# xbpeng/DeepMimic

Measured on NVIDIA H100. Metric: env-steps/sec (30 Hz policy steps; humanoid3d_spinkick, 4096 envs/GPU), higher is better.
Workload: dtype f32

## Files before the change

deepmimic_b200/capi.py:

```python
import ctypes as C
import os

import numpy as np

_REPO = os.path.dirname(os.path.dirname(os.path.abspath(__file__)))
_LIB_PATH = os.environ.get("DM_LIB", os.path.join(_REPO, "deepmimic_b200", "libdeepmimic_b200.so"))
_lib = None


class DmDims(C.Structure):
    _fields_ = [(n, C.c_int) for n in ("num_envs", "num_joints", "pose_dim", "num_dofs", "state_size", "goal_size", "action_size", "snapshot_size",
                                        "updates_per_action", "num_update_substeps")] + [("motion_duration", C.c_double), ("amp_obs_size", C.c_int)]


_fp = C.POINTER(C.c_float)


class DmMlpGatedWeights(C.Structure):
    _fields_ = ([(n, C.c_int) for n in ("in_dim", "goal_dim", "h0", "h1", "out_dim", "gate_common", "gate_hidden")]
                + [(n, _fp) for n in ("w0", "b0", "w1", "b1", "w2", "b2", "gc_w", "gc_b")]
                + [(n, _fp * 2) for n in ("gh_w", "gh_b", "gs_w", "gs_b", "gb_w", "gb_b")]
                + [(n, _fp) for n in ("s_mean", "s_std", "g_mean", "g_std", "a_mean", "a_std")] + [("s_clip", C.c_float), ("g_clip", C.c_float)])


# ... 14 lines not shown
                + [(n, C.c_float) for n in ("stepsize", "momentum", "weight_decay", "logit_reg_weight", "grad_penalty_weight")] + [("stats", C.c_void_p)])


class DmLearnGatedNet(C.Structure):
    _fields_ = [(n, C.c_void_p * 10) for n in ("w", "b", "acc_w", "acc_b")]


class DmLearnGatedBatch(C.Structure):
    _anonymous_ = ("batch",)
    _fields_ = [("batch", DmLearnBatch), ("goals", C.c_void_p), ("g_mean", C.c_void_p), ("g_istd", C.c_void_p), ("g_clip", C.c_float)]


DM_STATE_OFFSET, DM_STATE_SCALE, DM_ACTION_OFFSET, DM_ACTION_SCALE, DM_ACTION_BOUND_MIN, DM_ACTION_BOUND_MAX, DM_STATE_NORM_GROUPS = range(7)

EXPORTS = ["dm_create", "dm_load_host", "dm_plan_launch", "dm_get_model_info", "dm_get_link_table", "dm_destroy", "dm_last_error", "dm_get_dims", "dm_get_static", "dm_get_scene_name", "dm_stream", "dm_sync", "dm_set_mode", "dm_set_sample_count", "dm_get_time_limits", "dm_reset", "dm_set_action",
           "dm_update", "dm_set_env_order", "dm_plan_env_order", "dm_get_env_order", "dm_record_state", "dm_record_goal", "dm_goal_host", "dm_reset_clips", "dm_record_amp_obs_expert_clips", "dm_get_clip_table", "dm_get_task_state", "dm_set_task_state", "dm_get_task_params", "dm_calc_reward", "dm_calc_reward_imitate", "dm_record_amp_obs_agent", "dm_record_amp_obs_expert", "dm_amp_obs_host", "dm_sample_amp_obs_expert", "dm_expert_sample_count", "dm_observe", "dm_get_flags", "dm_step_host", "dm_step_host_reset", "dm_set_time_limits", "dm_exchange_create", "dm_exchange_connect", "dm_exchange_publish", "dm_exchange_acquire", "dm_exchange_release", "dm_exchange_status", "dm_exchange_destroy", "dm_set_timing", "dm_step_host_timing", "dm_get_snapshot",
           "dm_set_snapshot", "dm_state_size", "dm_save_state", "dm_load_state", "dm_get_counters", "dm_get_section_profile", "dm_mlp_create", "dm_mlp_forward", "dm_mlp_create_gated", "dm_mlp_forward_gated",
           "dm_mlp_forward_style_reward", "dm_mlp_launches", "dm_mlp_destroy", "dm_td_lambda_returns", "dm_mlp_set_weights_device", "dm_learn_create",
           "dm_mlp_set_normalizers_device", "dm_learn_set_weights", "dm_learn_step", "dm_learn_disc_step", "dm_learn_destroy",
           "dm_learn_create_gated", "dm_learn_set_gated_weights", "dm_learn_gated_step", "dm_mlp_set_gated_weights_device", "dm_mlp_set_gated_normalizers_device"]


def lib():
    global _lib
    if _lib is None:
        if not os.path.exists(_LIB_PATH):
            raise RuntimeError("deepmimic_b200: %s is missing -- run `python -c 'import __graft_entry__ as g; g.build()'`. "
                               "There is no CPU fallback." % _LIB_PATH)
        L = C.CDLL(_LIB_PATH)
        vp, dp, fp, ip = C.c_void_p, C.POINTER(C.c_double), C.c_void_p, C.c_void_p
        L.dm_create.restype = vp
# ... 8 lines not shown
        L.dm_get_dims.argtypes = [vp, C.POINTER(DmDims)]
        L.dm_get_static.argtypes = [vp, C.c_int, dp]
        L.dm_get_scene_name.argtypes = [vp, C.c_char_p, C.c_int]
        L.dm_stream.restype = vp
        L.dm_stream.argtypes = [vp]
        L.dm_sync.argtypes = [vp]
        L.dm_set_mode.argtypes = [vp, C.c_int]
        L.dm_set_sample_count.argtypes = [vp, C.c_longlong]
        L.dm_get_time_limits.argtypes = [vp, dp]
        L.dm_reset.argtypes = [vp, C.c_int, dp, dp, dp]
        L.dm_set_action.argtypes = [vp, fp]
        L.dm_update.argtypes = [vp, C.c_double, C.c_int]
        L.dm_set_env_order.argtypes = [vp, C.c_int]
        L.dm_plan_env_order.argtypes = [C.POINTER(C.c_int), C.c_int, C.c_int, C.c_int, C.POINTER(C.c_int)]
        L.dm_get_env_order.argtypes = [vp, C.POINTER(C.c_int), C.POINTER(C.c_int), C.POINTER(C.c_int)]
        L.dm_record_state.argtypes = [vp, fp]
        L.dm_record_goal.argtypes = [vp, fp]
        L.dm_calc_reward.argtypes = [vp, fp]
        L.dm_calc_reward_imitate.argtypes = [vp, fp]
        L.dm_goal_host.argtypes = [vp, fp]
        L.dm_reset_clips.argtypes = [vp, C.c_int, C.POINTER(C.c_int), dp, dp, dp]
        L.dm_record_amp_obs_expert_clips.argtypes = [vp, C.POINTER(C.c_int), dp, fp]
        L.dm_get_clip_table.argtypes = [vp, C.POINTER(C.c_int), dp, dp]
        L.dm_get_task_state.argtypes = [vp, C.c_int, dp]
        L.dm_set_task_state.argtypes = [vp, C.c_int, dp]
        L.dm_get_task_params.argtypes = [vp, dp, C.POINTER(C.c_uint64)]
        L.dm_record_amp_obs_agent.argtypes = [vp, fp]
        L.dm_record_amp_obs_expert.argtypes = [vp, dp, fp]
        L.dm_amp_obs_host.argtypes = [vp, C.c_int, dp, fp]
        L.dm_sample_amp_obs_expert.argtypes = [vp, C.c_int, vp, vp, vp]
# ... 150 lines not shown

    def update(self, dt, n_updates=1):
        self._chk(lib().dm_update(self.h, dt, n_updates))

    def set_env_order(self, on):
        self._chk(lib().dm_set_env_order(self.h, 1 if on else 0))

    def env_order(self):
        ip = C.POINTER(C.c_int)
        plan = np.zeros(3, dtype=np.int32)
        self._chk(lib().dm_get_env_order(self.h, plan.ctypes.data_as(ip), None, None))
        keys, order = np.zeros(plan[0], dtype=np.int32), np.zeros(plan[0], dtype=np.int32)
        self._chk(lib().dm_get_env_order(self.h, plan.ctypes.data_as(ip), keys.ctypes.data_as(ip), order.ctypes.data_as(ip)))
        return keys, order, int(plan[1]), int(plan[2])

    def observe(self, state=None, reward=None):
        self._chk(lib().dm_observe(self.h, C.c_void_p(state.data_ptr()) if state is not None else None,
                                   C.c_void_p(reward.data_ptr()) if reward is not None else None))

    def reward_imitate(self, out):
        self._chk(lib().dm_calc_reward_imitate(self.h, C.c_void_p(out.data_ptr())))

    def record_goal(self, out):
        self._chk(lib().dm_record_goal(self.h, C.c_void_p(out.data_ptr())))

    def goal_host(self):
        out = np.zeros((self.num_envs, self.dims.goal_size), dtype=np.float32)
        self._chk(lib().dm_goal_host(self.h, C.c_void_p(out.ctypes.data)))
        return out

# ... 121 lines not shown

    def load_state(self, buf):
        b = np.ascontiguousarray(buf, dtype=np.uint8)
        if b.ndim != 1 or b.size < 24 or int(b[16:24].view(np.uint64)[0]) != b.size:
            raise ValueError("load_state: not a complete save_state() blob (%s bytes)" % (b.shape,))
        self._chk(lib().dm_load_state(self.h, C.c_void_p(b.ctypes.data)))

    def counters(self):
        out = (C.c_int64 * 2)()
        self._chk(lib().dm_get_counters(self.h, out))
        return int(out[0]), int(out[1])

    def section_profile(self):
        nb, nw = C.c_int(0), C.c_int(0)
        self._chk(lib().dm_get_section_profile(self.h, None, C.byref(nb), C.byref(nw)))
        out = np.zeros((nb.value, nw.value, 18), dtype=np.uint32)
        self._chk(lib().dm_get_section_profile(self.h, C.c_void_p(out.ctypes.data), None, None))
        return out

    def stream(self):
        return lib().dm_stream(self.h)


class HostModel:
    INFO = dict(parents=0, joint_types=1, dof_offsets=2, pose_offsets=3, fall_bodies=4, end_effectors=5)

    def __init__(self, args, asset_root):
        L = lib()
        enc = [a.encode() for a in args]
        arr = (C.c_char_p * len(enc))(*enc)
        h = L.dm_load_host(asset_root.encode(), len(enc), arr)
# ... 282 lines not shown
```

deepmimic_b200/csrc/capi.cu:

```cuda
#include <cuda_runtime.h>

#include <algorithm>
#include <map>
#include <mutex>
#include <cmath>
#include <cstddef>
#include <cstdio>
#include <cstdlib>
#include <numeric>
#include <cstring>
#include <ctime>
#include <utility>
#include <memory>
#include <string>
#include <vector>

#include "../../include/deepmimic_b200.h"
#include "host/assets.hpp"
#include "kernels/dm_model.cuh"

namespace dmk {
__global__ void dm_flags_kernel(DevState st, int32_t* out, int num_real_envs) {
    int e = blockIdx.x * blockDim.x + threadIdx.x;
    if (e >= num_real_envs) return;
// ... 52 lines not shown
    double* d_frame_times = nullptr;
    float* d_frames = nullptr;
    float* d_frame_vel = nullptr;
    double* d_inj[3] = {nullptr, nullptr, nullptr};
    int32_t* d_flags4 = nullptr;
    float *d_amp = nullptr, *p_amp = nullptr;
    float *d_goal = nullptr, *p_goal = nullptr;
    dmk::ClipTable ctab{};
    dmk::ClipTable* d_ctab = nullptr; int* d_clip_inj = nullptr;
    int total_frames = 0;
    float *d_act = nullptr, *d_obs = nullptr, *d_rew = nullptr;
    float *p_act = nullptr, *p_obs = nullptr, *p_rew = nullptr; int32_t* p_flags = nullptr;
    cudaStream_t stream = nullptr;
    int device = 0, num_envs = 0, padded_envs = 0, W = 32, tiles = 2, maxrows = 36, smem_bytes = 0, mode = 0;
    int* d_order = nullptr;
    dmk::StepLayout lay{};
    uint64_t seed = 0, env_offset = 0;
    int64_t launches = 0;
    uint64_t amp_calls = 0;
    uint64_t expert_samples = 0;
    std::vector<double> st_off, st_scale, act_off, act_scale, act_min, act_max, st_groups;
    std::vector<std::pair<const void*, bool>> pin_cache;
    int x_rank = 0, x_world = 0;
    char* x_base = nullptr;
    char* x_peer[8] = {nullptr, nullptr, nullptr, nullptr, nullptr, nullptr, nullptr, nullptr};
    size_t x_data_off = 0, x_parity_bytes = 0;
    bool timing = false;
    cudaEvent_t tev[5] = {nullptr, nullptr, nullptr, nullptr, nullptr};
    double host_ms[3] = {0, 0, 0};
    std::vector<void*> dev_bufs, pinned_bufs;
// ... 222 lines not shown

int launch_step(dm_handle* h, double dt, int n_updates) {
    const dmk::StepKernel kern = dmk::kStepKernels[tile_index(h)][task_scene(h)];
    static std::mutex mu;
    static std::map<std::pair<int, const void*>, int> configured;
    {
        std::lock_guard<std::mutex> lock(mu);
        int& have = configured[{h->device, reinterpret_cast<const void*>(kern)}];
        if (h->smem_bytes > have) {
            DM_CUDA(cudaFuncSetAttribute(kern, cudaFuncAttributeMaxDynamicSharedMemorySize, h->smem_bytes));
            DM_CUDA(cudaFuncSetAttribute(kern, cudaFuncAttributePreferredSharedMemoryCarveout, 100));
            DM_CUDA(cudaFuncSetAttribute(dmk::dm_env_order_kernel, cudaFuncAttributePreferredSharedMemoryCarveout, 100));
            have = h->smem_bytes;
        }
    }
    if (h->st.order) {
        dmk::dm_env_order_kernel<<<1, dmk::kEnvOrderThreads, 0, h->stream>>>(h->st.load, h->padded_envs, h->tiles, h->W, h->d_order);
        if (launched(h)) return 1;
    }
    kern<<<h->padded_envs / h->tiles, h->tiles * h->W, h->smem_bytes, h->stream>>>(h->d_model, h->st, h->d_frame_times, h->d_frames, dt, n_updates,
                                                                                   h->sa.cfg.num_sim_substeps, h->lay);
    return launched(h);
}
int launch_observe_fan(dm_handle* h, const dmk::ObsFan& fan) {
    const dmk::ObserveKernel kern = dmk::kObserveKernels[tile_index(h)][task_scene(h)];
    const size_t smem = static_cast<size_t>(dmk::kPolicyBlock / h->W) * h->hm.state_size * sizeof(float);
    kern<<<policy_grid(h), dmk::kPolicyBlock, smem, h->stream>>>(h->d_model, h->st, h->d_frame_times, h->d_frames, h->d_frame_vel, fan, h->num_envs);
    return launched(h);
}
int launch_observe(dm_handle* h, float* d_state, float* d_reward) {
    dmk::ObsFan fan{};
    fan.n = 1; fan.obs[0] = d_state; fan.rew[0] = d_reward; fan.done[0] = nullptr;
    return launch_observe_fan(h, fan);
}
int launch_reset(dm_handle* h, int force, const double* kt, const double* mt, const double* th, const int* clip) {
    const dmk::ResetKernel kern = dmk::kResetKernels[tile_index(h)][task_scene(h)];
// ... 71 lines not shown
    auto even_split = [&](int slots, int cap) {
        const int waves = ((num_envs + cap - 1) / cap + slots - 1) / slots;
        int t = std::min(cap, std::max(min_tiles, (num_envs + waves * slots - 1) / (waves * slots)));
        if (H.W == 16 && (t & 1)) t = (t + 1 <= cap) ? t + 1 : t - 1;
        return std::make_pair(waves, t);
    };
    auto [waves, tiles] = even_split(sms, max_tiles);
    {
        const int cap2 = std::min({max_tiles, (smem_sm / 2 - smem_reserved - hot) / per_env, 65536 / (2 * regs * H.W)});
        if (cap2 >= min_tiles) {
            const auto [waves2, tiles2] = even_split(2 * sms, cap2);
            if (waves2 < waves) { waves = waves2; tiles = tiles2; }
        }
    }
    H.tiles = tiles;
    const int quantum = (tiles * (64 / H.W)) / std::__gcd(tiles, 64 / H.W);
    H.padded_envs = ((num_envs + quantum - 1) / quantum) * quantum;
    H.smem_bytes = dmk::dm_step_smem_bytes(H.lay, H.tiles) + 1024;
    return true;
}

extern "C" {

const char* dm_last_error(void) { return g_err.c_str(); }
void dm_set_last_error(const char* msg) { g_err = msg ? msg : ""; }

static bool load_host_model(dm_handle& H, const char* asset_root, int argc, const char** argv) {
    try {
        std::vector<std::string> args(argv, argv + argc);
        dmh::ArgParser ap;
// ... 109 lines not shown
        h->ctab.cdf[c] = h->sa.clip_cdf[c];
        ci.is_getup = std::find(h->sa.cfg.getup_motion_ids.begin(), h->sa.cfg.getup_motion_ids.end(), static_cast<int>(c)) != h->sa.cfg.getup_motion_ids.end() ? 1 : 0;
        h->total_frames += mc.num_frames;
    }
    const size_t TF = static_cast<size_t>(h->total_frames);
    DM_CUDA(cudaStreamCreateWithFlags(&h->stream, cudaStreamNonBlocking));
    if (alloc_buffer(h, &h->d_model, 1) || alloc_buffer(h, &h->st.sim, N * ss) || alloc_buffer(h, &h->st.time, N * dmk::kTimeDoubles, kZeroed) ||
        alloc_buffer(h, &h->st.flags, N * dmk::kFlagInts, kZeroed) || alloc_buffer(h, &h->st.manifold, N * M.nl * dmk::kManifoldFloats, kZeroed) ||
        alloc_buffer(h, &h->d_frame_times, TF) || alloc_buffer(h, &h->d_frames, TF * M.pose_dim) || alloc_buffer(h, &h->d_frame_vel, TF * M.pose_dim) ||
        alloc_buffer(h, &h->d_flags4, N * 4) || alloc_buffer(h, &h->d_amp, N * M.amp_obs_size) || alloc_buffer(h, &h->p_amp, N * M.amp_obs_size, kPinned) ||
        alloc_buffer(h, &h->st.hist, N * 2 * M.pose_dim, kZeroed) || alloc_buffer(h, &h->d_act, N * std::max(1, M.action_size)) ||
        alloc_buffer(h, &h->d_obs, N * M.state_size) || alloc_buffer(h, &h->d_rew, N) || alloc_buffer(h, &h->p_act, N * std::max(1, M.action_size), kPinned) ||
        alloc_buffer(h, &h->p_obs, N * M.state_size, kPinned) || alloc_buffer(h, &h->p_rew, N, kPinned) || alloc_buffer(h, &h->p_flags, N * 4, kPinned))
        return 1;
    for (auto& p : h->d_inj) if (alloc_buffer(h, &p, N)) return 1;
    if (alloc_buffer(h, &h->st.load, N) || alloc_buffer(h, &h->d_order, N)) return 1;
    {
        std::vector<int> load(N, 0), ident(N);
        std::fill(load.begin() + h->num_envs, load.end(), dmk::kLoadPadding);
        std::iota(ident.begin(), ident.end(), 0);
        DM_CUDA(cudaMemcpy(h->st.load, load.data(), N * sizeof(int), cudaMemcpyHostToDevice));
        DM_CUDA(cudaMemcpy(h->d_order, ident.data(), N * sizeof(int), cudaMemcpyHostToDevice));
    }
    h->st.order = (h->W == 16) ? h->d_order : nullptr;
#ifdef DM_PROFILE
    if (alloc_buffer(h, &h->st.prof, static_cast<size_t>(h->padded_envs / h->tiles) * (h->tiles * h->W / 32) * dmk::kProfCounters, kZeroed)) return 1;
#endif
    h->st.num_envs = h->padded_envs; h->st.num_real = h->num_envs;
    if (task_scene(h)) {
        if (alloc_buffer(h, &h->st.task, N * dmk::kTaskDoubles, kZeroed) || alloc_buffer(h, &h->st.taskx, N * dmk::kTaskExtDoubles, kZeroed) ||
            alloc_buffer(h, &h->d_goal, N * 4) || alloc_buffer(h, &h->p_goal, N * 4, kPinned) || alloc_buffer(h, &h->st.clip, N, kZeroed) ||
            alloc_buffer(h, &h->d_clip_inj, N) || alloc_buffer(h, &h->d_ctab, 1))
            return 1;
        DM_CUDA(cudaMemcpy(h->d_ctab, &h->ctab, sizeof(dmk::ClipTable), cudaMemcpyHostToDevice));
    }
    h->st.ctab = h->d_ctab;
    std::vector<float> frames(TF * M.pose_dim), fvel(frames.size());
    std::vector<double> ftimes(TF);
    for (size_t c = 0; c < h->sa.clips.size(); ++c) {
        const dmh::MotionClip& mc = h->sa.clips[c];
        const std::vector<double> fv = build_frame_vel(h->sa.character, mc);
// ... 147 lines not shown
        return fail();
    }
    std::vector<int> sorted(n_padded);
    std::iota(sorted.begin(), sorted.end(), 0);
    std::stable_sort(sorted.begin(), sorted.end(), [&](int a, int b) { return dmk::env_load_bucket(keys[a]) < dmk::env_load_bucket(keys[b]); });
    for (int r = 0; r < n_padded; ++r) order[dmk::env_order_slot(r, n_padded, tiles, W)] = sorted[r];
    return 0;
}
int dm_get_env_order(dm_handle* h, int* h_plan3, int* h_keys, int* h_order) {
    DM_DEVICE(h);
    if (h_plan3) { h_plan3[0] = h->padded_envs; h_plan3[1] = h->tiles; h_plan3[2] = h->W; }
    DM_CUDA(cudaStreamSynchronize(h->stream));
    if (h_keys) DM_CUDA(cudaMemcpy(h_keys, h->st.load, sizeof(int) * h->padded_envs, cudaMemcpyDeviceToHost));
    if (h_order && h->st.order) DM_CUDA(cudaMemcpy(h_order, h->st.order, sizeof(int) * h->padded_envs, cudaMemcpyDeviceToHost));
    else if (h_order) std::iota(h_order, h_order + h->padded_envs, 0);
    return 0;
}
static int launch_task_observe(dm_handle* h, float* d_goal, float* d_reward) {
    dmk::dm_task_observe_kernel<<<(h->num_envs + 127) / 128, 128, 0, h->stream>>>(h->d_model, h->st, d_goal, d_reward, h->num_envs);
    return launched(h);
}
int dm_observe(dm_handle* h, float* d_state, float* d_reward) {
    DM_DEVICE(h);
    const bool task = task_scene(h);
    float* d_imitate_reward = task ? nullptr : d_reward;
    if ((d_state != nullptr || d_imitate_reward != nullptr) && launch_observe(h, d_state, d_imitate_reward)) return 1;
    if (task && d_reward != nullptr) return launch_task_observe(h, nullptr, d_reward);
    return 0;
}
int dm_record_state(dm_handle* h, float* d_out) { return dm_observe(h, d_out, nullptr); }
// ... 443 lines not shown
    DM_CUDA(cudaStreamSynchronize(h->stream));
    h->amp_calls = in.amp_calls; h->expert_samples = in.expert_samples;
    h->hm.time_lim_min = in.time_lim_min; h->hm.time_lim_max = in.time_lim_max;
    if (upload_time_limits(h)) return 1;
    return dm_set_mode(h, in.mode);
}

int dm_get_section_profile(dm_handle* h, uint32_t* out, int* num_blocks, int* warps_per_block) {
    DM_DEVICE(h);
    if (!h->st.prof) { g_err = "dm_get_section_profile: this library is not the profile build (make -C deepmimic_b200/csrc profile)"; return fail(); }
    const int blocks = h->padded_envs / h->tiles, warps = h->tiles * h->W / 32;
    if (num_blocks) *num_blocks = blocks;
    if (warps_per_block) *warps_per_block = warps;
    if (out) {
        DM_CUDA(cudaStreamSynchronize(h->stream));
        DM_CUDA(cudaMemcpy(out, h->st.prof, static_cast<size_t>(blocks) * warps * dmk::kProfCounters * sizeof(uint32_t), cudaMemcpyDeviceToHost));
    }
    return 0;
}
int dm_get_counters(dm_handle* h, int64_t* out) {
    DM_DEVICE(h);
    DM_CUDA(cudaStreamSynchronize(h->stream));
    std::vector<int> fl(static_cast<size_t>(h->padded_envs) * dmk::kFlagInts);
    DM_CUDA(cudaMemcpy(fl.data(), h->st.flags, fl.size() * sizeof(int), cudaMemcpyDeviceToHost));
    int64_t over = 0;
    for (int e = 0; e < h->num_envs; ++e) over += fl[static_cast<size_t>(e) * dmk::kFlagInts + dmk::kFRowOverflow];
    out[0] = h->launches; out[1] = over;
    return 0;
}

}
// ... 1 lines not shown
```

deepmimic_b200/csrc/kernels/dm_model.cuh:

```cuda
#pragma once
#include <cstdint>

#include "dm_math.cuh"

#include "dm_task.cuh"
#include "dm_task_ext.cuh"

namespace dmk {

constexpr int kMaxLinks = 32;
constexpr int kMaxDofs = 96;
constexpr int kMaxChain = 24;
constexpr int kMaxChildren = 4;
constexpr int kStepMaxThreads = 448;
constexpr int kStepRegs = 128;
constexpr int kManifoldFloats = 48;
constexpr int kProfCounters = 18;

enum DevJointType { kJRevolute = 0, kJSpherical = 1, kJFixed = 2 };
enum DevShape { kSBox = 1, kSCapsule = 2, kSSphere = 3 };

struct DevLink {
    int parent, jtype, ndof, dof0;
    int level, nchild, child[kMaxChildren];
    int depth0;
    int last_depth;
    int shape, fall_contact, end_eff, has_limit;
    uint32_t anc_mask;
    float mass;
    float inertiaB[3];
    float inertiaD[3];
    float dvec[3], evec[3];
// ... 74 lines not shown
    double* time;
    int* flags;
    float* manifold;
    float* hist;
    unsigned int* prof;
    double* task;
    double* taskx;
    int* clip;
    const ClipTable* ctab;
    int num_envs;
    int num_real;
    int* load;
    const int* order;
};

constexpr int kLoadPadding = -1;
constexpr int kLoadBuckets = 64;
__host__ __device__ inline int env_load_bucket(int key) { const int b = kLoadBuckets - 2 - key; return b < 0 ? 0 : (b >= kLoadBuckets ? kLoadBuckets - 1 : b); }
__host__ __device__ inline int env_order_slot(int r, int n_padded, int tiles, int W) {
    const int per_warp = 32 / W, blocks = n_padded / tiles, warps = tiles / per_warp;
    const int g = r / per_warp, round = g / blocks, j = g % blocks;
    const int b = (round & 1) ? blocks - 1 - j : j;
    return (b * warps + round) * per_warp + r % per_warp;
}

constexpr int kMaxFan = 8;
struct ObsFan {
    int n;
    float* obs[kMaxFan];
    float* rew[kMaxFan];
// ... 10 lines not shown

constexpr int kPolicyBlock = 64;
using StepKernel = void (*)(const DevModel*, DevState, const double*, const float*, double, int, int, StepLayout);
using ObserveKernel = void (*)(const DevModel*, DevState, const double*, const float*, const float*, ObsFan, int);
using ResetKernel = void (*)(const DevModel*, DevState, const double*, const float*, const float*, int, const double*, const double*, const double*,
                             unsigned long long, unsigned long long, int, const int*);
using AmpObsKernel = void (*)(const DevModel*, DevState, const double*, const float*, const float*, float*, int, const double*, int, const int*);
extern const StepKernel kStepKernels[2][2];
extern const ObserveKernel kObserveKernels[2][2];
extern const ResetKernel kResetKernels[2][2];
extern const AmpObsKernel kAmpObsKernels[2][2];
using AmpExpertKernel = void (*)(const DevModel*, DevState, const double*, const float*, const float*, float*, int, unsigned long long, unsigned long long,
                                 int*, double*);
extern const AmpExpertKernel kAmpExpertKernels[2][2];
constexpr int kEnvOrderThreads = 1024;
__global__ void dm_env_order_kernel(const int* load, int n_padded, int tiles, int W, int* order);
__global__ void dm_set_action_kernel(const DevModel*, DevState, const float*, int);
__global__ void dm_task_reset_kernel(const DevModel*, DevState, int);
__global__ void dm_task_observe_kernel(const DevModel*, DevState, float*, float*, int);
int dm_step_layout(int nl, int n, int chain_len, int maxrows, int W, StepLayout* L);
int dm_step_smem_bytes(const StepLayout& L, int tiles);

}
```

deepmimic_b200/csrc/kernels/dm_step.cu:

```cuda
#include "dm_model.cuh"
#include <type_traits>

namespace dmk {

namespace {

template <int W>
struct Tl {
    static __device__ __forceinline__ float shfl(float v, int src) { return __shfl_sync(0xffffffffu, v, src, W); }
    static __device__ __forceinline__ int shfli(int v, int src) { return __shfl_sync(0xffffffffu, v, src, W); }
    static __device__ __forceinline__ V3 shfl3(V3 v, int src) { return mk3(shfl(v.x, src), shfl(v.y, src), shfl(v.z, src)); }
    static __device__ __forceinline__ S6 shfl6(S6 v, int src) { return mks(shfl3(v.a, src), shfl3(v.l, src)); }
};
__device__ __forceinline__ void ld12(const float* p, float* o) {
    const float4 a = reinterpret_cast<const float4*>(p)[0], b = reinterpret_cast<const float4*>(p)[1], c_ = reinterpret_cast<const float4*>(p)[2];
    o[0] = a.x; o[1] = a.y; o[2] = a.z; o[3] = a.w; o[4] = b.x; o[5] = b.y; o[6] = b.z; o[7] = b.w; o[8] = c_.x; o[9] = c_.y; o[10] = c_.z; o[11] = c_.w;
}
__device__ __forceinline__ void st12(float* p, const float* o) {
    reinterpret_cast<float4*>(p)[0] = make_float4(o[0], o[1], o[2], o[3]); reinterpret_cast<float4*>(p)[1] = make_float4(o[4], o[5], o[6], o[7]);
    reinterpret_cast<float4*>(p)[2] = make_float4(o[8], o[9], o[10], o[11]);
}
__device__ __forceinline__ float rcp_fast(float x) { float r; asm("rcp.approx.ftz.f32 %0, %1;" : "=f"(r) : "f"(x)); return r; }
__device__ __forceinline__ int wmax(int v) {
#pragma unroll
// ... 49 lines not shown
    return mkq(r.x * n, r.y * n, r.z * n, r.w * n);
}

enum LkSlot { kLC = 0 , kLM = 3,
              kLD = 4 , kLThr = 7,
              kLWd = 8 , kLInt = 14 , kLInt2 = 15 ,
              kLWb = 16 , kLFlg = 22 , kLTree = 23 ,
              kLAx = 24 , kLTl = 27,
              kLZr = 28 ,
              kLHe = 32 , kLKp = 35,
              kLKd = 36, kLLo = 37, kLHi = 38, kLChild = 39 ,
              kLDc = 40 , kLMc = 43 ,
              kLDyn = 44 , kLDChild = 45 ,
              kLkFloats = 48 };
__device__ __forceinline__ float4 ld4(const float* p) { return *reinterpret_cast<const float4*>(p); }
enum HdrSlot { kHLayout = 0, kHLvc = 24, kHGrav = 32 , kHh = 35, kHScale = 36, kHMu = 37, kHFdt = 38, kHDmax = 39 , kHdrFloats = 40 };
__device__ __forceinline__ float* step_smem() { extern __shared__ __align__(16) float dm_step_sm[]; return dm_step_sm; }

}

int dm_step_layout(int nl, int n, int chain_len, int maxrows, int W, StepLayout* L) {
    const int maxpts = maxrows / 3;
    int o = 0;
    L->nl = nl; L->n = n; L->chain_len = chain_len; L->maxrows = maxrows; L->maxpts = maxpts;
    L->oU = o; o += nl * 24;
    L->oR = o; o += nl * 12;
    L->oA = o;
    const int world = nl * 24, tri = maxrows * (maxrows + 1) / 2;
    L->oW = o; L->oV = o + nl * 12;
    L->oPp = o + world; L->oQ = L->oPp + maxpts * 4;
    const int pre = world + maxpts * 4 + 4 * 8;
// ... 863 lines not shown
    if (c.jtype == kJSpherical) jww = jvx * S0 + jvy * S1 + jvz * S2; else if (c.jtype == kJRevolute) jww = jvx * S0;
    S6 vel = mks(mk3(0, 0, 0), mk3(0, 0, 0));
    if (c.lane == 0) { const V3 bo = mk3(sB[7], sB[8], sB[9]); vel = mks(bo + jww, mk3(sB[10], sB[11], sB[12]) + cross(bo, cw)); }
#pragma unroll 1
    for (int lv = 1; lv <= c.maxlevel; ++lv) {
        const S6 pv = T::shfl6(vel, c.plane);
        if (c.level == lv) vel = mks(pv.a + jww, pv.l + cross(pv.a, cw));
    }
    if (c.act && want) {
        float* v = sV + c.lane * 12;
        v[0] = vel.a.x; v[1] = vel.a.y; v[2] = vel.a.z; v[3] = vel.l.x; v[4] = vel.l.y; v[5] = vel.l.z;
    }
    __syncwarp();
}

template <int W, bool TASK>
__global__ void __launch_bounds__(kStepMaxThreads, 1) dm_step_kernel(const DevModel* __restrict__ gm, DevState st, const double* __restrict__ frame_times,
                                                                       const float* __restrict__ frames, double dt, int n_updates, int sim_substeps, StepLayout LY) {
    using T = Tl<W>;
    extern __shared__ __align__(16) float sm[];
    const int tiles = blockDim.x / W;
    const int tile = threadIdx.x / W;
    const int lane = threadIdx.x % W;
    const int slot = blockIdx.x * tiles + tile;
    const int env = (W == 16 && st.order) ? st.order[slot] : slot;
    const DevModel& M = *gm;
    const int nl = LY.nl, CL = LY.chain_len;
    const bool act = lane < nl;
    const int li = act ? lane : nl - 1;

    float* LK = sm + kHdrFloats;
    unsigned char* CD = reinterpret_cast<unsigned char*>(LK + nl * kLkFloats);
    unsigned char* CH = CD + nl * nl;
    int* LYS = reinterpret_cast<int*>(sm + kHLayout);
    for (int j = threadIdx.x; j < nl; j += blockDim.x) {
        const DevLink& K = M.link[j];
        float* q = LK + j * kLkFloats;
        const int p = K.parent;
        for (int k = 0; k < 3; ++k) { q[kLC + k] = K.evec[k] + (p >= 0 ? M.link[p].dvec[k] : 0.f); q[kLD + k] = K.dvec[k]; q[kLAx + k] = K.axis[k]; }
        q[kLM] = K.mass;
// ... 39 lines not shown
        reinterpret_cast<int*>(q)[kLInt2] = (K.dof0 & 0xff) | ((K.last_depth & 0xff) << 8) | ((K.nchild & 0xff) << 16);
        for (int k = 0; k < 4; ++k) q[kLZr + k] = K.zrot[k];
        for (int k = 0; k < 3; ++k) q[kLHe + k] = K.he[k];
        q[kLThr] = K.break_thr; q[kLKp] = K.kp; q[kLKd] = K.kd; q[kLTl] = K.tlim; q[kLLo] = K.lim_lo; q[kLHi] = K.lim_hi;
        reinterpret_cast<int*>(q)[kLFlg] = (K.shape & 0xff) | ((K.fall_contact & 0xff) << 8) | ((K.has_limit & 0xff) << 16);
        reinterpret_cast<int*>(q)[kLTree] = (K.level & 0xff) | ((M.maxlevel & 0xff) << 8) | ((K.nchild & 0xff) << 16);
        reinterpret_cast<int*>(q)[kLChild] = (K.child[0] & 0xff) | ((K.child[1] & 0xff) << 8) | ((K.child[2] & 0xff) << 16) | ((K.child[3] & 0xff) << 24);
        for (int d = 0; d < CL; ++d) CH[j * CL + d] = M.chain_dof[j][d];
        for (int b = 0; b < nl; ++b) {
            int cnt = 0;
            const int lim = min(K.last_depth, M.link[b].last_depth);
            while (cnt <= lim && M.chain_dof[j][cnt] == M.chain_dof[b][cnt]) ++cnt;
            CD[j * nl + b] = static_cast<unsigned char>(cnt);
        }
    }
    if (threadIdx.x == blockDim.x - 1) {
        static_assert(sizeof(StepLayout) / sizeof(int) <= kHLvc, "StepLayout must fit the header slot");
        const int* src = reinterpret_cast<const int*>(&LY);
        for (int k = 0; k < static_cast<int>(sizeof(StepLayout) / sizeof(int)); ++k) LYS[k] = src[k];
        sm[kHGrav] = M.gravity[0]; sm[kHGrav + 1] = M.gravity[1]; sm[kHGrav + 2] = M.gravity[2];
        sm[kHh] = static_cast<float>(dt) / static_cast<float>(sim_substeps); sm[kHScale] = M.scale; sm[kHMu] = M.friction; sm[kHFdt] = static_cast<float>(dt);
    }
    if (threadIdx.x == 8) {
        int mx = 0;
        for (int j = 0; j < nl; ++j) { const DevLink& K = M.link[j]; if (K.parent >= 0 && !(K.ndof == 0 && K.nchild == 0 && M.link[K.parent].ndof > 0)) mx = max(mx, K.level - 1); }
        reinterpret_cast<int*>(sm)[kHDmax] = mx;
    }
    __syncthreads();

    float* E = sm + LY.hot_floats + tile * LY.env_floats;
    for (int k = lane * 4; k < LY.env_floats; k += W * 4) *reinterpret_cast<float4*>(E + k) = make_float4(0.f, 0.f, 0.f, 0.f);
    __syncwarp();
    float* sV = E + LY.oV; float* sG = E + LY.oG; float* sQ = E + LY.oQ; float* sLam = E + LY.oLam;
    const float* LKo = LK + li * kLkFloats;
    const int jtype = (reinterpret_cast<const int*>(LKo)[kLInt] >> 8) & 0xff, ndof = act ? ((reinterpret_cast<const int*>(LKo)[kLInt] >> 16) & 0xff) : 0;
    const int lflags = reinterpret_cast<const int*>(LKo)[kLFlg];
    const bool fall_contact = ((lflags >> 8) & 0xff) != 0, has_limit = ((lflags >> 16) & 0xff) != 0;

    const int ss = sim_stride(nl);
    float* sim = st.sim + static_cast<size_t>(env) * ss;
    double* tm = st.time + static_cast<size_t>(env) * kTimeDoubles;
    int* fl = st.flags + static_cast<size_t>(env) * kFlagInts;
    float* mani = st.manifold + static_cast<size_t>(env) * nl * kManifoldFloats;
// ... 261 lines not shown
        PROF(2);
        if (lane == 0) {
            sB[0] += h * sB[10]; sB[1] += h * sB[11]; sB[2] += h * sB[12];
            const Q4 q = quat_integrate3(mk3(sB[7], sB[8], sB[9]), mkq(sB[3], sB[4], sB[5], sB[6]), true, h);
            sB[3] = q.x; sB[4] = q.y; sB[5] = q.z; sB[6] = q.w;
        }
        if (jtype == kJRevolute) jp.x += h * jv.x;
        else if (jtype == kJSpherical) { Q4 q = quat_integrate3(mk3(jv.x, jv.y, jv.z), mkq(jp.x, jp.y, jp.z, jp.w), false, h); jp = make_float4(q.x, q.y, q.z, q.w); }
        __syncwarp();
        need_kin = true;
        if (ph == sim_substeps) pending_flags = true;
        PROF(12);
    }
#ifdef DM_PROFILE
    __syncwarp();
    if ((threadIdx.x & 31) == 0 && st.prof) { unsigned int* o = st.prof + (blockIdx.x * (blockDim.x / 32) + threadIdx.x / 32) * kProfCounters; for (int k = 0; k < kProfCounters; ++k) o[k] = PRF[k]; }
#endif
}

const StepKernel kStepKernels[2][2] = {{dm_step_kernel<16, false>, dm_step_kernel<16, true>}, {dm_step_kernel<32, false>, dm_step_kernel<32, true>}};

constexpr int kEnvOrderItems = 4;
__global__ void __launch_bounds__(kEnvOrderThreads) dm_env_order_kernel(const int* __restrict__ load, int n_padded, int tiles, int W, int* __restrict__ order) {
    constexpr int kWarps = kEnvOrderThreads / 32, kCells = kEnvOrderItems * kWarps, kChunk = kEnvOrderItems * kEnvOrderThreads;
    constexpr int kParts = kEnvOrderThreads / kLoadBuckets, kPer = kCells / kParts;
    static_assert(kParts <= 32 && 32 % kParts == 0 && kCells % kParts == 0, "the scan of a bucket's cells runs inside one warp");
    __shared__ int base[kLoadBuckets];
    __shared__ int cnt[kLoadBuckets][kCells + 1];
    const int t = threadIdx.x, warp = t / 32, lane = t % 32;
    const unsigned lt = (1u << lane) - 1u;
    int b[kEnvOrderItems];
    auto load_chunk = [&](int c0) {
#pragma unroll
        for (int i = 0; i < kEnvOrderItems; ++i) { const int e = c0 + i * kEnvOrderThreads + t; b[i] = (e < n_padded) ? env_load_bucket(load[e]) : kLoadBuckets; }
    };
    auto count = [&](int bk) {
        const unsigned peers = __match_any_sync(0xffffffffu, bk);
        if (bk < kLoadBuckets && (peers & lt) == 0) atomicAdd(&base[bk], __popc(peers));
// ... 52 lines not shown
```

include/deepmimic_b200.h:

```cpp
#ifndef DEEPMIMIC_B200_H_
#define DEEPMIMIC_B200_H_
#include <stddef.h>
#include <stdint.h>
#ifdef __cplusplus
extern "C" {
#endif

typedef struct dm_handle dm_handle;

typedef struct dm_dims {
    int num_envs;
    int num_joints;
    int pose_dim;
    int num_dofs;
    int state_size;
    int goal_size;
    int action_size;
    int snapshot_size;
    int updates_per_action;
    int num_update_substeps;
    double motion_duration;
    int amp_obs_size;
} dm_dims;

// ... 17 lines not shown
int dm_get_scene_name(dm_handle* h, char* h_out, int capacity);
int dm_get_static(dm_handle* h, int kind, double* h_out);
void* dm_stream(dm_handle* h);
int dm_sync(dm_handle* h);
int dm_set_mode(dm_handle* h, int mode);
int dm_set_sample_count(dm_handle* h, long long count);
int dm_set_time_limits(dm_handle* h, double t_min, double t_max);
int dm_get_time_limits(dm_handle* h, double* h_out3);

int dm_reset(dm_handle* h, int force_all, const double* h_kin_time, const double* h_max_time, const double* h_rot_theta);
int dm_set_action(dm_handle* h, const float* d_actions);
int dm_update(dm_handle* h, double dt, int n_updates);
int dm_set_env_order(dm_handle* h, int on);
int dm_plan_env_order(const int* keys, int n_padded, int tiles, int W, int* order);
int dm_get_env_order(dm_handle* h, int* h_plan3, int* h_keys, int* h_order);
int dm_record_state(dm_handle* h, float* d_out);
int dm_record_goal(dm_handle* h, float* d_out);
int dm_goal_host(dm_handle* h, float* h_out);
int dm_reset_clips(dm_handle* h, int force_all, const int* h_clip, const double* h_kin_time, const double* h_max_time, const double* h_rot_theta);
int dm_record_amp_obs_expert_clips(dm_handle* h, const int* h_clip, const double* h_kin_time, float* d_out);
int dm_get_clip_table(dm_handle* h, int* num_clips, double* h_dur, double* h_cdf);
int dm_get_task_state(dm_handle* h, int env, double* h_out16);
int dm_set_task_state(dm_handle* h, int env, const double* h_in16);
int dm_get_task_params(dm_handle* h, double* h_out48, unsigned long long* h_stream2);
int dm_calc_reward(dm_handle* h, float* d_out);
int dm_calc_reward_imitate(dm_handle* h, float* d_out);
int dm_record_amp_obs_agent(dm_handle* h, float* d_out);
int dm_record_amp_obs_expert(dm_handle* h, const double* h_kin_time, float* d_out);
int dm_amp_obs_host(dm_handle* h, int expert, const double* h_kin_time, float* h_out);
int dm_sample_amp_obs_expert(dm_handle* h, int rows, float* d_out, int* d_clip_out, double* d_time_out);
// ... 107 lines not shown
```

Before: 2.518 million.

## Schedule heaviest env blocks onto lone SMs and overlap order kernel via PDL

Adds a dynamic block placement step in the step kernel: each CTA registers its SM id, waits briefly for all CTAs to arrive, then blocks alone on an SM take the heaviest env slots from the front while shared SMs take slots from the back. The sorted env order plus this mapping aims to balance load when the grid runs in a single wave. The step kernel is also launched with programmatic stream serialization, so its prologue overlaps the env-order kernel and waits at griddepcontrol.wait. In exchange it adds a spin-wait with a timeout, global atomics, and extra scheduling words in the order buffer.

Result: faster. 2.554 million, median of 6 (+1.4%).

```diff
diff --git a/deepmimic_b200/capi.py b/deepmimic_b200/capi.py
--- a/deepmimic_b200/capi.py
+++ b/deepmimic_b200/capi.py
@@ -52,7 +52,7 @@
 DM_STATE_OFFSET, DM_STATE_SCALE, DM_ACTION_OFFSET, DM_ACTION_SCALE, DM_ACTION_BOUND_MIN, DM_ACTION_BOUND_MAX, DM_STATE_NORM_GROUPS = range(7)
 
 EXPORTS = ["dm_create", "dm_load_host", "dm_plan_launch", "dm_get_model_info", "dm_get_link_table", "dm_destroy", "dm_last_error", "dm_get_dims", "dm_get_static", "dm_get_scene_name", "dm_stream", "dm_sync", "dm_set_mode", "dm_set_sample_count", "dm_get_time_limits", "dm_reset", "dm_set_action",
-           "dm_update", "dm_set_env_order", "dm_plan_env_order", "dm_get_env_order", "dm_record_state", "dm_record_goal", "dm_goal_host", "dm_reset_clips", "dm_record_amp_obs_expert_clips", "dm_get_clip_table", "dm_get_task_state", "dm_set_task_state", "dm_get_task_params", "dm_calc_reward", "dm_calc_reward_imitate", "dm_record_amp_obs_agent", "dm_record_amp_obs_expert", "dm_amp_obs_host", "dm_sample_amp_obs_expert", "dm_expert_sample_count", "dm_observe", "dm_get_flags", "dm_step_host", "dm_step_host_reset", "dm_set_time_limits", "dm_exchange_create", "dm_exchange_connect", "dm_exchange_publish", "dm_exchange_acquire", "dm_exchange_release", "dm_exchange_status", "dm_exchange_destroy", "dm_set_timing", "dm_step_host_timing", "dm_get_snapshot",
+           "dm_update", "dm_set_env_order", "dm_plan_env_order", "dm_get_env_order", "dm_set_block_schedule", "dm_get_block_schedule", "dm_record_state", "dm_record_goal", "dm_goal_host", "dm_reset_clips", "dm_record_amp_obs_expert_clips", "dm_get_clip_table", "dm_get_task_state", "dm_set_task_state", "dm_get_task_params", "dm_calc_reward", "dm_calc_reward_imitate", "dm_record_amp_obs_agent", "dm_record_amp_obs_expert", "dm_amp_obs_host", "dm_sample_amp_obs_expert", "dm_expert_sample_count", "dm_observe", "dm_get_flags", "dm_step_host", "dm_step_host_reset", "dm_set_time_limits", "dm_exchange_create", "dm_exchange_connect", "dm_exchange_publish", "dm_exchange_acquire", "dm_exchange_release", "dm_exchange_status", "dm_exchange_destroy", "dm_set_timing", "dm_step_host_timing", "dm_get_snapshot",
            "dm_set_snapshot", "dm_state_size", "dm_save_state", "dm_load_state", "dm_get_counters", "dm_get_section_profile", "dm_mlp_create", "dm_mlp_forward", "dm_mlp_create_gated", "dm_mlp_forward_gated",
            "dm_mlp_forward_style_reward", "dm_mlp_launches", "dm_mlp_destroy", "dm_td_lambda_returns", "dm_mlp_set_weights_device", "dm_learn_create",
            "dm_mlp_set_normalizers_device", "dm_learn_set_weights", "dm_learn_step", "dm_learn_disc_step", "dm_learn_destroy",
@@ -91,6 +91,8 @@
         L.dm_set_env_order.argtypes = [vp, C.c_int]
         L.dm_plan_env_order.argtypes = [C.POINTER(C.c_int), C.c_int, C.c_int, C.c_int, C.POINTER(C.c_int)]
         L.dm_get_env_order.argtypes = [vp, C.POINTER(C.c_int), C.POINTER(C.c_int), C.POINTER(C.c_int)]
+        L.dm_set_block_schedule.argtypes = [vp, C.c_int]
+        L.dm_get_block_schedule.argtypes = [vp, C.POINTER(C.c_int), C.POINTER(C.c_int)]
         L.dm_record_state.argtypes = [vp, fp]
         L.dm_record_goal.argtypes = [vp, fp]
         L.dm_calc_reward.argtypes = [vp, fp]
@@ -271,6 +273,18 @@
         self._chk(lib().dm_get_env_order(self.h, plan.ctypes.data_as(ip), keys.ctypes.data_as(ip), order.ctypes.data_as(ip)))
         return keys, order, int(plan[1]), int(plan[2])
 
+    def set_block_schedule(self, on):
+        self._chk(lib().dm_set_block_schedule(self.h, 1 if on else 0))
+
+    def block_schedule(self):
+        ip = C.POINTER(C.c_int)
+        plan = np.zeros(3, dtype=np.int32)
+        self._chk(lib().dm_get_env_order(self.h, plan.ctypes.data_as(ip), None, None))
+        on = C.c_int(0)
+        m = np.zeros((plan[0] // plan[1], 3), dtype=np.int32)
+        self._chk(lib().dm_get_block_schedule(self.h, C.byref(on), m.ctypes.data_as(ip)))
+        return bool(on.value), m
+
     def observe(self, state=None, reward=None):
         self._chk(lib().dm_observe(self.h, C.c_void_p(state.data_ptr()) if state is not None else None,
                                    C.c_void_p(reward.data_ptr()) if reward is not None else None))
@@ -422,7 +436,7 @@
     def section_profile(self):
         nb, nw = C.c_int(0), C.c_int(0)
         self._chk(lib().dm_get_section_profile(self.h, None, C.byref(nb), C.byref(nw)))
-        out = np.zeros((nb.value, nw.value, 18), dtype=np.uint32)
+        out = np.zeros((nb.value, nw.value, 22), dtype=np.uint32)
         self._chk(lib().dm_get_section_profile(self.h, C.c_void_p(out.ctypes.data), None, None))
         return out
 
diff --git a/deepmimic_b200/csrc/capi.cu b/deepmimic_b200/csrc/capi.cu
--- a/deepmimic_b200/csrc/capi.cu
+++ b/deepmimic_b200/csrc/capi.cu
@@ -90,6 +90,9 @@
     cudaStream_t stream = nullptr;
     int device = 0, num_envs = 0, padded_envs = 0, W = 32, tiles = 2, maxrows = 36, smem_bytes = 0, mode = 0;
     int* d_order = nullptr;
+    bool one_wave = false;
+    bool block_schedule = true;
+    bool scheduled = false;
     dmk::StepLayout lay{};
     uint64_t seed = 0, env_offset = 0;
     int64_t launches = 0;
@@ -342,12 +345,19 @@
             have = h->smem_bytes;
         }
     }
+    h->scheduled = h->st.order && h->block_schedule && h->one_wave;
     if (h->st.order) {
-        dmk::dm_env_order_kernel<<<1, dmk::kEnvOrderThreads, 0, h->stream>>>(h->st.load, h->padded_envs, h->tiles, h->W, h->d_order);
+        dmk::dm_env_order_kernel<<<1, dmk::kEnvOrderThreads, 0, h->stream>>>(h->st.load, h->padded_envs, h->tiles, h->W, h->d_order, h->scheduled ? 1 : 0);
         if (launched(h)) return 1;
     }
-    kern<<<h->padded_envs / h->tiles, h->tiles * h->W, h->smem_bytes, h->stream>>>(h->d_model, h->st, h->d_frame_times, h->d_frames, dt, n_updates,
-                                                                                   h->sa.cfg.num_sim_substeps, h->lay);
+    cudaLaunchAttribute dep{};
+    dep.id = cudaLaunchAttributeProgrammaticStreamSerialization;
+    dep.val.programmaticStreamSerializationAllowed = 1;
+    cudaLaunchConfig_t cfg{};
+    cfg.gridDim = dim3(h->padded_envs / h->tiles); cfg.blockDim = dim3(h->tiles * h->W); cfg.dynamicSmemBytes = h->smem_bytes; cfg.stream = h->stream;
+    cfg.attrs = &dep; cfg.numAttrs = h->st.order ? 1 : 0;
+    DM_CUDA(cudaLaunchKernelEx(&cfg, kern, static_cast<const dmk::DevModel*>(h->d_model), h->st, static_cast<const double*>(h->d_frame_times),
+                               static_cast<const float*>(h->d_frames), dt, n_updates, h->sa.cfg.num_sim_substeps, h->lay));
     return launched(h);
 }
 int launch_observe_fan(dm_handle* h, const dmk::ObsFan& fan) {
@@ -449,6 +459,7 @@
         }
     }
     H.tiles = tiles;
+    H.one_wave = waves == 1;
     const int quantum = (tiles * (64 / H.W)) / std::__gcd(tiles, 64 / H.W);
     H.padded_envs = ((num_envs + quantum - 1) / quantum) * quantum;
     H.smem_bytes = dmk::dm_step_smem_bytes(H.lay, H.tiles) + 1024;
@@ -588,17 +599,17 @@
         alloc_buffer(h, &h->p_obs, N * M.state_size, kPinned) || alloc_buffer(h, &h->p_rew, N, kPinned) || alloc_buffer(h, &h->p_flags, N * 4, kPinned))
         return 1;
     for (auto& p : h->d_inj) if (alloc_buffer(h, &p, N)) return 1;
-    if (alloc_buffer(h, &h->st.load, N) || alloc_buffer(h, &h->d_order, N)) return 1;
+    if (alloc_buffer(h, &h->st.load, N) || alloc_buffer(h, &h->d_order, N + dmk::sched_words(h->padded_envs / h->tiles))) return 1;
     {
-        std::vector<int> load(N, 0), ident(N);
+        std::vector<int> load(N, 0), ident(N + dmk::sched_words(h->padded_envs / h->tiles), 0);
         std::fill(load.begin() + h->num_envs, load.end(), dmk::kLoadPadding);
-        std::iota(ident.begin(), ident.end(), 0);
+        std::iota(ident.begin(), ident.begin() + N, 0);
         DM_CUDA(cudaMemcpy(h->st.load, load.data(), N * sizeof(int), cudaMemcpyHostToDevice));
-        DM_CUDA(cudaMemcpy(h->d_order, ident.data(), N * sizeof(int), cudaMemcpyHostToDevice));
+        DM_CUDA(cudaMemcpy(h->d_order, ident.data(), ident.size() * sizeof(int), cudaMemcpyHostToDevice));
     }
     h->st.order = (h->W == 16) ? h->d_order : nullptr;
 #ifdef DM_PROFILE
-    if (alloc_buffer(h, &h->st.prof, static_cast<size_t>(h->padded_envs / h->tiles) * (h->tiles * h->W / 32) * dmk::kProfCounters, kZeroed)) return 1;
+    if (alloc_buffer(h, &h->st.prof, static_cast<size_t>(h->padded_envs / h->tiles) * (h->tiles * h->W / 32) * dmk::kProfWords, kZeroed)) return 1;
 #endif
     h->st.num_envs = h->padded_envs; h->st.num_real = h->num_envs;
     if (task_scene(h)) {
@@ -776,6 +787,20 @@
     if (h_keys) DM_CUDA(cudaMemcpy(h_keys, h->st.load, sizeof(int) * h->padded_envs, cudaMemcpyDeviceToHost));
     if (h_order && h->st.order) DM_CUDA(cudaMemcpy(h_order, h->st.order, sizeof(int) * h->padded_envs, cudaMemcpyDeviceToHost));
     else if (h_order) std::iota(h_order, h_order + h->padded_envs, 0);
+    return 0;
+}
+int dm_set_block_schedule(dm_handle* h, int on) {
+    DM_DEVICE(h);
+    h->block_schedule = on != 0;
+    return 0;
+}
+int dm_get_block_schedule(dm_handle* h, int* h_scheduled, int* h_map) {
+    DM_DEVICE(h);
+    DM_CUDA(cudaStreamSynchronize(h->stream));
+    if (h_scheduled) *h_scheduled = h->scheduled ? 1 : 0;
+    const int blocks = h->padded_envs / h->tiles;
+    if (h_map && h->scheduled) DM_CUDA(cudaMemcpy(h_map, h->d_order + h->padded_envs + dmk::kSchMap, sizeof(int) * 3 * blocks, cudaMemcpyDeviceToHost));
+    else if (h_map) for (int b = 0; b < blocks; ++b) { h_map[3 * b] = b; h_map[3 * b + 1] = -1; h_map[3 * b + 2] = -1; }
     return 0;
 }
 static int launch_task_observe(dm_handle* h, float* d_goal, float* d_reward) {
@@ -1249,7 +1274,7 @@
     if (warps_per_block) *warps_per_block = warps;
     if (out) {
         DM_CUDA(cudaStreamSynchronize(h->stream));
-        DM_CUDA(cudaMemcpy(out, h->st.prof, static_cast<size_t>(blocks) * warps * dmk::kProfCounters * sizeof(uint32_t), cudaMemcpyDeviceToHost));
+        DM_CUDA(cudaMemcpy(out, h->st.prof, static_cast<size_t>(blocks) * warps * dmk::kProfWords * sizeof(uint32_t), cudaMemcpyDeviceToHost));
     }
     return 0;
 }
diff --git a/deepmimic_b200/csrc/kernels/dm_model.cuh b/deepmimic_b200/csrc/kernels/dm_model.cuh
--- a/deepmimic_b200/csrc/kernels/dm_model.cuh
+++ b/deepmimic_b200/csrc/kernels/dm_model.cuh
@@ -16,6 +16,8 @@
 constexpr int kStepRegs = 128;
 constexpr int kManifoldFloats = 48;
 constexpr int kProfCounters = 18;
+constexpr int kProfWords = kProfCounters + 4;
+enum ProfPlacement { kPrSmid = kProfCounters, kPrLone, kPrCta, kPrPrologue };
 
 enum DevJointType { kJRevolute = 0, kJSpherical = 1, kJFixed = 2 };
 enum DevShape { kSBox = 1, kSCapsule = 2, kSSphere = 3 };
@@ -120,6 +122,11 @@
     const int* order;
 };
 
+constexpr int kSchedSMs = 256;
+constexpr int kSchedWaitNs = 5000;
+enum SchedWord { kSchOn = 0, kSchArrivals, kSchFront, kSchBack, kSchPerSM, kSchMap = kSchPerSM + kSchedSMs };
+__host__ __device__ constexpr int sched_words(int blocks) { return kSchMap + 3 * blocks; }
+
 constexpr int kLoadPadding = -1;
 constexpr int kLoadBuckets = 64;
 __host__ __device__ inline int env_load_bucket(int key) { const int b = kLoadBuckets - 2 - key; return b < 0 ? 0 : (b >= kLoadBuckets ? kLoadBuckets - 1 : b); }
@@ -160,7 +167,7 @@
                                  int*, double*);
 extern const AmpExpertKernel kAmpExpertKernels[2][2];
 constexpr int kEnvOrderThreads = 1024;
-__global__ void dm_env_order_kernel(const int* load, int n_padded, int tiles, int W, int* order);
+__global__ void dm_env_order_kernel(const int* load, int n_padded, int tiles, int W, int* order, int schedule);
 __global__ void dm_set_action_kernel(const DevModel*, DevState, const float*, int);
 __global__ void dm_task_reset_kernel(const DevModel*, DevState, int);
 __global__ void dm_task_observe_kernel(const DevModel*, DevState, float*, float*, int);
diff --git a/deepmimic_b200/csrc/kernels/dm_step.cu b/deepmimic_b200/csrc/kernels/dm_step.cu
--- a/deepmimic_b200/csrc/kernels/dm_step.cu
+++ b/deepmimic_b200/csrc/kernels/dm_step.cu
@@ -87,7 +87,7 @@
               kLDyn = 44 , kLDChild = 45 ,
               kLkFloats = 48 };
 __device__ __forceinline__ float4 ld4(const float* p) { return *reinterpret_cast<const float4*>(p); }
-enum HdrSlot { kHLayout = 0, kHLvc = 24, kHGrav = 32 , kHh = 35, kHScale = 36, kHMu = 37, kHFdt = 38, kHDmax = 39 , kHdrFloats = 40 };
+enum HdrSlot { kHLayout = 0, kHBlock = 24, kHLone = 25, kHGrav = 32 , kHh = 35, kHScale = 36, kHMu = 37, kHFdt = 38, kHDmax = 39 , kHdrFloats = 40 };
 __device__ __forceinline__ float* step_smem() { extern __shared__ __align__(16) float dm_step_sm[]; return dm_step_sm; }
 
 }
@@ -981,6 +981,31 @@
     __syncwarp();
 }
 
+__device__ __forceinline__ unsigned int sm_id() { unsigned int r; asm volatile("mov.u32 %0, %%smid;" : "=r"(r)); return r; }
+__device__ __forceinline__ unsigned int ld_volatile(const unsigned int* p) { return *reinterpret_cast<const volatile unsigned int*>(p); }
+__device__ __noinline__ void sched_place(unsigned int* S, int* hdr) {
+    int b = blockIdx.x, lone = 2;
+    if (ld_volatile(S + kSchOn) != 0) {
+        const unsigned int smid = sm_id();
+        if (smid < kSchedSMs) atomicAdd(S + kSchPerSM + smid, 1u);
+        __threadfence();
+        atomicAdd(S + kSchArrivals, 1u);
+        unsigned long long t0, t1;
+        asm volatile("mov.u64 %0, %%globaltimer;" : "=l"(t0));
+        while (ld_volatile(S + kSchArrivals) < gridDim.x) {
+            asm volatile("mov.u64 %0, %%globaltimer;" : "=l"(t1));
+            if (t1 - t0 > kSchedWaitNs) break;
+            __nanosleep(100);
+        }
+        __threadfence();
+        lone = (smid < kSchedSMs && ld_volatile(S + kSchPerSM + smid) == 1u) ? 1 : 0;
+        b = lone ? static_cast<int>(atomicAdd(S + kSchFront, 1u)) : static_cast<int>(gridDim.x) - 1 - static_cast<int>(atomicAdd(S + kSchBack, 1u));
+        unsigned int* m = S + kSchMap + 3 * b;
+        m[0] = blockIdx.x; m[1] = smid; m[2] = static_cast<unsigned int>(lone);
+    }
+    hdr[kHBlock] = b; hdr[kHLone] = lone;
+}
+
 template <int W, bool TASK>
 __global__ void __launch_bounds__(kStepMaxThreads, 1) dm_step_kernel(const DevModel* __restrict__ gm, DevState st, const double* __restrict__ frame_times,
                                                                        const float* __restrict__ frames, double dt, int n_updates, int sim_substeps, StepLayout LY) {
@@ -989,8 +1014,9 @@
     const int tiles = blockDim.x / W;
     const int tile = threadIdx.x / W;
     const int lane = threadIdx.x % W;
-    const int slot = blockIdx.x * tiles + tile;
-    const int env = (W == 16 && st.order) ? st.order[slot] : slot;
+#ifdef DM_PROFILE
+    const unsigned int prf_entry = static_cast<unsigned int>(clock64());
+#endif
     const DevModel& M = *gm;
     const int nl = LY.nl, CL = LY.chain_len;
     const bool act = lane < nl;
@@ -1060,12 +1086,18 @@
             CD[j * nl + b] = static_cast<unsigned char>(cnt);
         }
     }
+    if constexpr (W == 16) asm volatile("griddepcontrol.wait;" ::: "memory");
     if (threadIdx.x == blockDim.x - 1) {
-        static_assert(sizeof(StepLayout) / sizeof(int) <= kHLvc, "StepLayout must fit the header slot");
+        static_assert(sizeof(StepLayout) / sizeof(int) <= kHBlock, "StepLayout must fit the header slot");
         const int* src = reinterpret_cast<const int*>(&LY);
         for (int k = 0; k < static_cast<int>(sizeof(StepLayout) / sizeof(int)); ++k) LYS[k] = src[k];
         sm[kHGrav] = M.gravity[0]; sm[kHGrav + 1] = M.gravity[1]; sm[kHGrav + 2] = M.gravity[2];
         sm[kHh] = static_cast<float>(dt) / static_cast<float>(sim_substeps); sm[kHScale] = M.scale; sm[kHMu] = M.friction; sm[kHFdt] = static_cast<float>(dt);
+        if constexpr (W == 16) {
+            int* hdr = reinterpret_cast<int*>(sm);
+            if (st.order) sched_place(reinterpret_cast<unsigned int*>(const_cast<int*>(st.order) + st.num_envs), hdr);
+            else { hdr[kHBlock] = blockIdx.x; hdr[kHLone] = 2; }
+        }
     }
     if (threadIdx.x == 8) {
         int mx = 0;
@@ -1073,6 +1105,13 @@
         reinterpret_cast<int*>(sm)[kHDmax] = mx;
     }
     __syncthreads();
+#ifdef DM_PROFILE
+    const unsigned int prf_prologue = static_cast<unsigned int>(clock64()) - prf_entry;
+#endif
+    int blk = blockIdx.x;
+    if constexpr (W == 16) blk = reinterpret_cast<const int*>(sm)[kHBlock];
+    const int slot = blk * tiles + tile;
+    const int env = (W == 16 && st.order) ? st.order[slot] : slot;
 
     float* E = sm + LY.hot_floats + tile * LY.env_floats;
     for (int k = lane * 4; k < LY.env_floats; k += W * 4) *reinterpret_cast<float4*>(E + k) = make_float4(0.f, 0.f, 0.f, 0.f);
@@ -1364,14 +1403,21 @@
     }
 #ifdef DM_PROFILE
     __syncwarp();
-    if ((threadIdx.x & 31) == 0 && st.prof) { unsigned int* o = st.prof + (blockIdx.x * (blockDim.x / 32) + threadIdx.x / 32) * kProfCounters; for (int k = 0; k < kProfCounters; ++k) o[k] = PRF[k]; }
+    if ((threadIdx.x & 31) == 0 && st.prof) {
+        unsigned int* o = st.prof + (blk * (blockDim.x / 32) + threadIdx.x / 32) * kProfWords;
+        for (int k = 0; k < kProfCounters; ++k) o[k] = PRF[k];
+        o[kPrSmid] = sm_id(); o[kPrLone] = (W == 16) ? reinterpret_cast<const int*>(sm)[kHLone] : 2; o[kPrCta] = blockIdx.x; o[kPrPrologue] = prf_prologue;
+    }
 #endif
 }
 
 const StepKernel kStepKernels[2][2] = {{dm_step_kernel<16, false>, dm_step_kernel<16, true>}, {dm_step_kernel<32, false>, dm_step_kernel<32, true>}};
 
 constexpr int kEnvOrderItems = 4;
-__global__ void __launch_bounds__(kEnvOrderThreads) dm_env_order_kernel(const int* __restrict__ load, int n_padded, int tiles, int W, int* __restrict__ order) {
+__global__ void __launch_bounds__(kEnvOrderThreads) dm_env_order_kernel(const int* __restrict__ load, int n_padded, int tiles, int W, int* __restrict__ order,
+                                                                        int schedule) {
+    asm volatile("griddepcontrol.launch_dependents;");
+    for (int k = threadIdx.x; k < sched_words(n_padded / tiles); k += kEnvOrderThreads) order[n_padded + k] = (k == kSchOn) ? schedule : (k < kSchMap ? 0 : -1);
     constexpr int kWarps = kEnvOrderThreads / 32, kCells = kEnvOrderItems * kWarps, kChunk = kEnvOrderItems * kEnvOrderThreads;
     constexpr int kParts = kEnvOrderThreads / kLoadBuckets, kPer = kCells / kParts;
     static_assert(kParts <= 32 && 32 % kParts == 0 && kCells % kParts == 0, "the scan of a bucket's cells runs inside one warp");
diff --git a/include/deepmimic_b200.h b/include/deepmimic_b200.h
--- a/include/deepmimic_b200.h
+++ b/include/deepmimic_b200.h
@@ -55,6 +55,8 @@
 int dm_set_env_order(dm_handle* h, int on);
 int dm_plan_env_order(const int* keys, int n_padded, int tiles, int W, int* order);
 int dm_get_env_order(dm_handle* h, int* h_plan3, int* h_keys, int* h_order);
+int dm_set_block_schedule(dm_handle* h, int on);
+int dm_get_block_schedule(dm_handle* h, int* h_scheduled, int* h_map);
 int dm_record_state(dm_handle* h, float* d_out);
 int dm_record_goal(dm_handle* h, float* d_out);
 int dm_goal_host(dm_handle* h, float* h_out);
```
